# Neela08/cloud-security-pytorch-sagemaker-distributed-workshop

Hardware: AMD Instinct MI355X
Metric: images/sec (whole node) ResNet-50 DDP (higher is better)
Workload: dtype bf16; 1 GPU; model=resnet50, global_batch=256, per_gpu_batch=256, image_size=224, parallelism=dp1, optimizer=SGD(momentum=0.9, wd=1e-4), fp32 master weights, bf16 compute, backend=none, launcher=none, device=cuda, comm_forced_at_world1=False, buckets=5, grad_comm=fp32, wgrad_stream=True, hip_graph=False, gpu_max_hw_queues=8

## Files before the change

### csrc/kernels/norm_act.hip

```cpp
#include "common.h"
#include <mutex>
#include <algorithm>
#include <cstdlib>

namespace {

constexpr int NT = 256;
constexpr bool kBnxNt = false;

struct SlabGeom {
  int tpr;
  int rp;
  int cw;
};

__host__ __device__ inline SlabGeom slab_geom(int C) {
  SlabGeom g;
  g.tpr = C / 8 < NT ? C / 8 : NT;
  g.rp = NT / g.tpr;
  g.cw = g.tpr * 8;
  return g;
}

__device__ __forceinline__ void block_reduce_store(float* s0, float* s1, float* part, int C, int cbase,
                                                   const SlabGeom& g) {
  __shared__ float red[2][NT * 8];
  const int tid = threadIdx.x;
  const int c8 = tid % g.tpr, r0 = tid / g.tpr;
#pragma unroll
  for (int j = 0; j < 8; ++j) {
    red[0][r0 * g.cw + c8 * 8 + j] = s0[j];
// ... 735 lines not shown
    *(float4*)&b[0] = *(const float4*)(shift + cc); *(float4*)&b[4] = *(const float4*)(shift + cc + 4);
#pragma unroll
    for (int j = 0; j < 8; ++j) { best[j] = -INFINITY; bi[j] = 0; }
#pragma unroll
    for (int tp = 0; tp < 9; ++tp) {
      if (!ok[tp]) continue;
      float f[8];
      unpack8(v[tp], f);
#pragma unroll
      for (int j = 0; j < 8; ++j) {
        const float val = bf2f(f2bf(fmaxf(f[j] * a[j] + b[j], 0.f)));
        if (val > best[j]) { best[j] = val; bi[j] = tp; }
      }
    }
    const size_t o = (size_t)t * 8;
    *(uint4*)(y + o) = pack8(best);
    uint2 packed;
    packed.x = bi[0] | (bi[1] << 8) | (bi[2] << 16) | (bi[3] << 24);
    packed.y = bi[4] | (bi[5] << 8) | (bi[6] << 16) | (bi[7] << 24);
    *(uint2*)(idx + o) = packed;
  }
}

__device__ __forceinline__ uint32_t tap_of(const uint2& ii, int j) {
  return ((j < 4 ? ii.x : ii.y) >> (8 * (j & 3))) & 0xffu;
}

__device__ __forceinline__ void bnpool3_quad(const bf16_t* __restrict__ dy, const uint8_t* __restrict__ idx,
                                             const bf16_t* __restrict__ c, const float* a, const float* b, int n,
                                             int p, int q, int cc, int H, int W, int C, int P, int Q, float dz[4][8],
                                             float cv[4][8], bool valid[4]) {
  const bool pn = p + 1 < P, qn = q + 1 < Q;
  const size_t o00 = (((size_t)n * P + p) * Q + q) * C + cc;
  const size_t o01 = qn ? o00 + C : o00, o10 = pn ? o00 + (size_t)Q * C : o00;
  const size_t o11 = (pn && qn) ? o00 + (size_t)Q * C + C : o00;
  const uint4 g00 = epi_ld16<kBnxNt>(dy + o00), g01 = epi_ld16<kBnxNt>(dy + o01);
  const uint4 g10 = epi_ld16<kBnxNt>(dy + o10), g11 = epi_ld16<kBnxNt>(dy + o11);
  const uint2 i00 = *(const uint2*)(idx + o00), i01 = *(const uint2*)(idx + o01);
  const uint2 i10 = *(const uint2*)(idx + o10), i11 = *(const uint2*)(idx + o11);
  const int h0 = 2 * p, w0 = 2 * q;
  uint4 xv[4];
#pragma unroll
  for (int i = 0; i < 4; ++i) {
    const int h = h0 + (i >> 1), w = w0 + (i & 1);
    valid[i] = h < H && w < W;
    xv[i] = epi_ld16<kBnxNt>(c + (((size_t)n * H + (valid[i] ? h : h0)) * W + (valid[i] ? w : w0)) * C + cc);
  }
  float f00[8], f01[8], f10[8], f11[8];
  unpack8(g00, f00); unpack8(g01, f01); unpack8(g10, f10); unpack8(g11, f11);
#pragma unroll
  for (int i = 0; i < 4; ++i) unpack8(xv[i], cv[i]);
#pragma unroll
  for (int j = 0; j < 8; ++j) {
    const uint32_t t00 = tap_of(i00, j), t01 = qn ? tap_of(i01, j) : 0xffu;
    const uint32_t t10 = pn ? tap_of(i10, j) : 0xffu, t11 = (pn && qn) ? tap_of(i11, j) : 0xffu;
    float acc[4];
    acc[0] = t00 == 4u ? f00[j] : 0.f;
    acc[1] = (t00 == 5u ? f00[j] : 0.f) + (t01 == 3u ? f01[j] : 0.f);
    acc[2] = (t00 == 7u ? f00[j] : 0.f) + (t10 == 1u ? f10[j] : 0.f);
    acc[3] = (t00 == 8u ? f00[j] : 0.f) + (t01 == 6u ? f01[j] : 0.f) + (t10 == 2u ? f10[j] : 0.f) +
             (t11 == 0u ? f11[j] : 0.f);
#pragma unroll
    for (int i = 0; i < 4; ++i) dz[i][j] = bf2f(f2bf(cv[i][j] * a[j] + b[j])) > 0.f ? acc[i] : 0.f;
  }
}

__global__ __launch_bounds__(NT) void bnpool3_bwd_stats_kernel(const bf16_t* __restrict__ dy,
                                                               const uint8_t* __restrict__ idx,
                                                               const bf16_t* __restrict__ c,
                                                               const float* __restrict__ scale,
                                                               const float* __restrict__ shift,
                                                               const float* __restrict__ mean,
                                                               float* __restrict__ part, int Nb, int H, int W, int C,
                                                               int P, int Q, int rows_per_block) {
  const SlabGeom g = slab_geom(C);
  const int tid = threadIdx.x;
  const int c8 = tid % g.tpr, r0 = tid / g.tpr;
  const int cbase = blockIdx.y * g.cw;
  const int cc = cbase + c8 * 8;
  const int M = Nb * P * Q;
  const int rb = blockIdx.x * rows_per_block, re = min(M, rb + rows_per_block);
  float a[8], b[8], mu[8];
#pragma unroll
  for (int j = 0; j < 8; ++j) { a[j] = scale[cc + j]; b[j] = shift[cc + j]; mu[j] = mean[cc + j]; }
  float sd[8] = {0}, sq[8] = {0};
  for (int r = rb + r0; r < re; r += g.rp) {
    const int q = r % Q, np = r / Q;
    const int p = np % P, n = np / P;
    float dz[4][8], cv[4][8];
    bool valid[4];
    bnpool3_quad(dy, idx, c, a, b, n, p, q, cc, H, W, C, P, Q, dz, cv, valid);
#pragma unroll
    for (int i = 0; i < 4; ++i) {
      if (!valid[i]) continue;
#pragma unroll
      for (int j = 0; j < 8; ++j) { sd[j] += dz[i][j]; sq[j] += dz[i][j] * (cv[i][j] - mu[j]); }
    }
  }
  block_reduce_store(sd, sq, part, C, cbase, g);
}

__global__ __launch_bounds__(NT) void bnpool3_bwd_apply_kernel(const bf16_t* __restrict__ dy,
                                                               const uint8_t* __restrict__ idx,
                                                               const bf16_t* __restrict__ c,
                                                               const float* __restrict__ scale,
                                                               const float* __restrict__ shift,
                                                               const float* __restrict__ coef,
                                                               bf16_t* __restrict__ dc, int H, int W, int C, int P,
                                                               int Q, int total) {
  const int C8 = C / 8;
  for (int t = blockIdx.x * NT + threadIdx.x; t < total; t += gridDim.x * NT) {
    const int c8 = t % C8;
    const int pix = t / C8;
    const int q = pix % Q, np = pix / Q;
    const int p = np % P, n = np / P;
    const int cc = c8 * 8;
    float a[8], b[8], k0[8], k1[8], k2[8];
    *(float4*)&a[0] = *(const float4*)(scale + cc); *(float4*)&a[4] = *(const float4*)(scale + cc + 4);
    *(float4*)&b[0] = *(const float4*)(shift + cc); *(float4*)&b[4] = *(const float4*)(shift + cc + 4);
    *(float4*)&k0[0] = *(const float4*)(coef + cc); *(float4*)&k0[4] = *(const float4*)(coef + cc + 4);
    *(float4*)&k1[0] = *(const float4*)(coef + C + cc); *(float4*)&k1[4] = *(const float4*)(coef + C + cc + 4);
    *(float4*)&k2[0] = *(const float4*)(coef + 2 * C + cc); *(float4*)&k2[4] = *(const float4*)(coef + 2 * C + cc + 4);
    float dz[4][8], cv[4][8];
    bool valid[4];
    bnpool3_quad(dy, idx, c, a, b, n, p, q, cc, H, W, C, P, Q, dz, cv, valid);
#pragma unroll
    for (int i = 0; i < 4; ++i) {
      if (!valid[i]) continue;
      float o[8];
#pragma unroll
      for (int j = 0; j < 8; ++j) o[j] = k0[j] * dz[i][j] + k1[j] * cv[i][j] + k2[j];
      *(uint4*)(dc + (((size_t)n * H + 2 * p + (i >> 1)) * W + 2 * q + (i & 1)) * C + cc) = pack8(o);
    }
  }
}

inline int ew_grid_cap() {
  static int cap = -1;
  if (cap < 0) {
    const char* e = std::getenv("MI355X_DP_EW_GRID_CAP");
    cap = (e && std::atoi(e) > 0) ? std::atoi(e) : kEwGridCap;
  }
  return cap;
}

inline int ew_grid(int64_t nvec) {
  int64_t g = (nvec + NT * EW_U - 1) / (NT * EW_U);
  const int cap = ew_grid_cap();
  return (int)(g < cap ? g : cap);
}

inline bool ew_fixc(int grid, int C) { return ((int64_t)grid * NT * 8) % C == 0; }

template <bool RES_BN>
inline void launch_bn_apply(const void* x, const void* res, void* y, const float* scale, const float* shift,
// ... 437 lines not shown

MI_API int mi_bnpool_fwd(const void* c, const float* scale, const float* shift, void* y, void* idx, int Nb, int H,
                         int W, int C, int P, int Q, int k, int s, int pad, hipStream_t st) {
  if (C % 8 || k * k > 255) return (int)hipErrorInvalidValue;
  const int64_t total = (int64_t)Nb * P * Q * (C / 8);
  const int64_t g = std::min<int64_t>((total + NT - 1) / NT, 16384);
  if (k == 3 && s == 2 && pad == 1 && total < INT32_MAX && (int64_t)Nb * H * W * C < INT32_MAX * 8ll) {
    hipLaunchKernelGGL(bnpool3_fwd_kernel, dim3((int)g), dim3(NT), 0, st, (const bf16_t*)c, scale, shift,
                       (bf16_t*)y, (uint8_t*)idx, H, W, C, P, Q, (int)total);
    return (int)hipGetLastError();
  }
  hipLaunchKernelGGL(bnpool_fwd_kernel, dim3((int)g), dim3(NT), 0, st, (const bf16_t*)c, scale, shift, (bf16_t*)y,
                     (uint8_t*)idx, Nb, H, W, C, P, Q, k, s, pad);
  return (int)hipGetLastError();
}

MI_API int mi_bnpool_bwd(const void* dy, const void* idx, const void* c, void* dc, int Nb, int H, int W, int C, int P,
                         int Q, int k, int s, int pad, const float* scale, const float* shift, const float* gamma,
                         const float* save_mean, const float* save_invstd, float* dgamma, float* dbeta, float* coef,
                         float* part, hipStream_t st) {
  if (C % 8 || k * k > 255) return (int)hipErrorInvalidValue;
  const int M = Nb * H * W;
  const bool k3 = k == 3 && s == 2 && pad == 1 && (int64_t)M * C < INT32_MAX;
  int nblk, rpb; dim3 grid;
  bnpool_launch_dims(k3 ? Nb * P * Q : M, C, nblk, rpb, grid);
  if (k3)
    hipLaunchKernelGGL(bnpool3_bwd_stats_kernel, grid, dim3(NT), 0, st, (const bf16_t*)dy, (const uint8_t*)idx,
                       (const bf16_t*)c, scale, shift, save_mean, part, Nb, H, W, C, P, Q, rpb);
  else
    hipLaunchKernelGGL(bnpool_bwd_stats_kernel, grid, dim3(NT), 0, st, (const bf16_t*)dy, (const uint8_t*)idx,
                       (const bf16_t*)c, scale, shift, save_mean, part, Nb, H, W, C, P, Q, k, s, pad, rpb);
  slab_finalize<true>(part, nblk, fin_bwd_args(M, C, gamma, save_mean, save_invstd, dgamma, dbeta, coef), st);
  if (k3) {
    const int total3 = Nb * P * Q * (C / 8);
    hipLaunchKernelGGL(bnpool3_bwd_apply_kernel, dim3(std::min(cdiv(total3, NT), 16384)), dim3(NT), 0, st,
                       (const bf16_t*)dy, (const uint8_t*)idx, (const bf16_t*)c, scale, shift, coef, (bf16_t*)dc, H,
                       W, C, P, Q, total3);
    return (int)hipGetLastError();
  }
  const int64_t total = (int64_t)M * (C / 8);
  const int64_t g = std::min<int64_t>((total + NT - 1) / NT, 16384);
  hipLaunchKernelGGL(bnpool_bwd_apply_kernel, dim3((int)g), dim3(NT), 0, st, (const bf16_t*)dy, (const uint8_t*)idx,
                     (const bf16_t*)c, scale, shift, coef, (bf16_t*)dc, Nb, H, W, C, P, Q, k, s, pad);
  return (int)hipGetLastError();
}
```

### csrc/kernels/stem_conv.hip

```cpp
#include "common.h"
#include <algorithm>
#include <cstdlib>

extern "C" float* mi_partials_workspace(size_t floats, hipStream_t st);

namespace {

constexpr int SR = 7, SS = 7, SSTR = 2;
constexpr int NTAP = SR * SS;
constexpr int KSTEPS = (NTAP + 3) / 4;
constexpr int KOUT = 64;
constexpr int ROWPX = 256;
constexpr int PAIR_ROWS = SSTR + SR;
constexpr int NEW_ROWS = 2 * SSTR;
constexpr int NRING = PAIR_ROWS + NEW_ROWS;
constexpr int MAX_BLOCKS = 256;
constexpr int STEM_T = 512;

struct StemArgs {
  const bf16_t* x;
  const bf16_t* w;
  bf16_t* y;
  float* stats;
  int Nb, H, W, P, Q, pad;
// ... 152 lines not shown
  }
  __syncthreads();
  if (tid < 2 * KOUT) {
    const int which = tid / KOUT, n = tid - which * KOUT;
    float t = 0.f;
#pragma unroll
    for (int w8 = 0; w8 < 8; ++w8) t += sred[(w8 * 2 + which) * KOUT + n];
    a.stats[((size_t)blockIdx.x * 2 + which) * KOUT + n] = t;
  }
}

constexpr int NUT = (NTAP + 1) / 2;
constexpr int DYPX = 128;
constexpr int STEM_WELEMS = KOUT * NTAP * 8;

struct StemWArgs {
  const bf16_t* x;
  const bf16_t* dy;
  float* dw;
  float* ws;
  int Nb, H, W, P, Q, pad;
  int pairs_per_img, total_pairs, pairs_per_block;
  int x_bytes, dy_bytes;
};

__device__ __forceinline__ int dy_swz(int px) { return (((px >> 1) & 1) << 1) | (((px >> 3) & 1) << 2); }

__global__ __launch_bounds__(STEM_T, 1) void stem_wgrad_kernel(StemWArgs a) {
  extern __shared__ __attribute__((aligned(16))) uint4 sm[];
  uint4* ring = sm;
  uint4* dys = sm + NRING * ROWPX;

  const int tid = threadIdx.x, lane = tid & 63, wid = tid >> 6;
  const int g = lane >> 4, li = lane & 15, q4 = li >> 2, p4 = li & 3;
  const int g0 = blockIdx.x * a.pairs_per_block;
  const int g1 = min(a.total_pairs, g0 + a.pairs_per_block);
  const int HC = (a.Q - 1) * SSTR + SS;

  const __amdgpu_buffer_rsrc_t rsx = __builtin_amdgcn_make_buffer_rsrc((void*)a.x, (short)0, a.x_bytes, 0x00020000);
  const __amdgpu_buffer_rsrc_t rsd = __builtin_amdgcn_make_buffer_rsrc((void*)a.dy, (short)0, a.dy_bytes, 0x00020000);
  constexpr uint32_t OOB = 0xFFFFFFF0u;

  auto load_rows = [&](int img, int ih0, int nrows) {
    for (int c = wid; c < nrows * 4; c += 8) {
      const int k = c >> 2, part = c & 3;
      const int ih = ih0 + k;
      const int pos = part * 64 + lane;
      const int px = pos < ROWPX / 2 ? 2 * pos : 2 * (pos - ROWPX / 2) + 1;
      const int iw = px - a.pad;
      const bool ok = px < HC && (unsigned)ih < (unsigned)a.H && (unsigned)iw < (unsigned)a.W;
      const uint32_t vo = ok ? (uint32_t)((((img * a.H + ih) * a.W + iw) * 8) * 2) : OOB;
      const int slot = (ih + a.pad) % NRING;
      __builtin_amdgcn_raw_ptr_buffer_load_lds(rsx, LDS_PTR(void, &ring[slot * ROWPX + part * 64]), 16, vo, 0, 0, 0);
    }
  };
  auto load_dy = [&](int img, int jp, int buf) {
    for (int c = wid; c < 2 * DYPX / 8; c += 8) {
      const int h = c / (DYPX / 8), px = (c % (DYPX / 8)) * 8 + (lane >> 3);
      const int p = 2 * jp + h;
      const int lc = (lane & 7) ^ dy_swz(px);
      const bool ok = px < a.Q && p < a.P;
      const uint32_t vo = ok ? (uint32_t)((((img * a.P + p) * a.Q + px) * KOUT + lc * 8) * 2) : OOB;
      __builtin_amdgcn_raw_ptr_buffer_load_lds(rsd, LDS_PTR(void, &dys[((buf * 2 + h) * DYPX + (c % (DYPX / 8)) * 8) * 8]),
                                               16, vo, 0, 0, 0);
    }
  };

  f32x4 acc[4][4];
#pragma unroll
  for (int m = 0; m < 4; ++m)
#pragma unroll
    for (int v = 0; v < 4; ++v) acc[m][v] = f32x4{0.f, 0.f, 0.f, 0.f};
  const int nv = wid + 24 < NUT ? 4 : 3;

  if (g0 < g1) {
    const int img = g0 / a.pairs_per_img, j = g0 - img * a.pairs_per_img;
    load_rows(img, 2 * SSTR * j - a.pad, PAIR_ROWS);
    load_dy(img, j, 0);
  }
  int buf = 0;
  const uint2* ring2 = (const uint2*)ring;
  const uint2* dys2 = (const uint2*)dys;
  for (int gp = g0; gp < g1; ++gp) {
    const int img = gp / a.pairs_per_img, jp = gp - img * a.pairs_per_img;
    asm volatile("s_waitcnt vmcnt(0)" ::: "memory");
    __syncthreads();
    const bool next_same = gp + 1 < g1 && (gp + 1) / a.pairs_per_img == img;
    if (next_same) {
      load_rows(img, 2 * SSTR * jp - a.pad + PAIR_ROWS, NEW_ROWS);
      load_dy(img, jp + 1, buf ^ 1);
    }
#pragma unroll
    for (int h = 0; h < 2; ++h) {
      const int p = 2 * jp + h;
      if (p >= a.P) continue;
      const int rbase = (SSTR * p) % NRING;
      for (int c = 0; c < DYPX / 32; ++c) {
        if (32 * c >= a.Q) break;
        const int px1 = 32 * c + 8 * g + q4, px2 = px1 + 4;
        bf16x8 af[4], bfr[4];
#pragma unroll
        for (int m = 0; m < 4; ++m) {
          const int lc = 2 * m + (p4 >> 1);
          const uint2* r1 = dys2 + ((buf * 2 + h) * DYPX + px1) * 16 + 2 * (lc ^ dy_swz(px1)) + (p4 & 1);
          const uint2* r2 = dys2 + ((buf * 2 + h) * DYPX + px2) * 16 + 2 * (lc ^ dy_swz(px2)) + (p4 & 1);
          short4v lo = __builtin_amdgcn_ds_read_tr16_b64_v4i16(LDS_PTR(short4v, r1));
          short4v hi = __builtin_amdgcn_ds_read_tr16_b64_v4i16(LDS_PTR(short4v, r2));
          short v8 __attribute__((ext_vector_type(8))) = {lo[0], lo[1], lo[2], lo[3], hi[0], hi[1], hi[2], hi[3]};
          af[m] = __builtin_bit_cast(bf16x8, v8);
        }
        const int qa = min(px1, a.Q - 1), qb = min(px2, a.Q - 1);
#pragma unroll
        for (int v = 0; v < 4; ++v) {
          if (v >= nv) break;
          const int u = wid + 8 * v;
          const int t = min(2 * u + (p4 >> 1), NTAP - 1);
          const int r = t / SS, sx = t - (t / SS) * SS;
          int slot = rbase + r;
          slot = slot >= NRING ? slot - NRING : slot;
          const int cb = slot * ROWPX + (sx & 1) * (ROWPX / 2) + (sx >> 1);
          short4v lo = __builtin_amdgcn_ds_read_tr16_b64_v4i16(LDS_PTR(short4v, ring2 + (cb + qa) * 2 + (p4 & 1)));
          short4v hi = __builtin_amdgcn_ds_read_tr16_b64_v4i16(LDS_PTR(short4v, ring2 + (cb + qb) * 2 + (p4 & 1)));
          short v8 __attribute__((ext_vector_type(8))) = {lo[0], lo[1], lo[2], lo[3], hi[0], hi[1], hi[2], hi[3]};
          bfr[v] = __builtin_bit_cast(bf16x8, v8);
        }
#pragma unroll
        for (int v = 0; v < 4; ++v) {
          if (v >= nv) break;
#pragma unroll
          for (int m = 0; m < 4; ++m)
            acc[m][v] = __builtin_amdgcn_mfma_f32_16x16x32_bf16(af[m], bfr[v], acc[m][v], 0, 0, 0);
        }
      }
    }
    buf ^= 1;
    if (gp + 1 < g1 && !next_same) {
      asm volatile("s_waitcnt vmcnt(0)" ::: "memory");
      __syncthreads();
      const int img2 = (gp + 1) / a.pairs_per_img, j2 = (gp + 1) - img2 * a.pairs_per_img;
      load_rows(img2, 2 * SSTR * j2 - a.pad, PAIR_ROWS);
      load_dy(img2, j2, buf);
    }
  }
  float* prow = a.ws ? a.ws + (size_t)blockIdx.x * STEM_WELEMS : nullptr;
#pragma unroll
  for (int v = 0; v < 4; ++v) {
    if (v >= nv) break;
    const int tap = 2 * (wid + 8 * v) + (li >> 3);
    if (tap >= NTAP) continue;
#pragma unroll
    for (int m = 0; m < 4; ++m)
#pragma unroll
      for (int r = 0; r < 4; ++r) {
        const int k = 16 * m + 4 * g + r;
        const size_t o = ((size_t)k * NTAP + tap) * 8 + (li & 7);
        if (prow) prow[o] = acc[m][v][r];
        else atomicAdd(a.dw + o, acc[m][v][r]);
      }
  }
}

constexpr int SWR_POS = 32, SWR_G = 8;
__global__ __launch_bounds__(256) void stem_wgrad_reduce_kernel(const float4* __restrict__ ws, float4* __restrict__ dw,
                                                                int rows) {
// ... 38 lines not shown
      float v[8];
#pragma unroll
      for (int u = 0; u < 8; ++u) v[u] = b + u * SWR_G < rows ? ws[(size_t)(b + u * SWR_G) * STEM_WELEMS + o] : 0.f;
#pragma unroll
      for (int u = 0; u < 8; ++u) s += v[u];
    }
  red[grp][pl] = s;
  __syncthreads();
  if (grp != 0 || pos >= ne) return;
  for (int gg = 1; gg < SWR_G; ++gg) s += red[gg][pl];
  float* d = g + k * sK + c * sC + (tap / SS) * sR + (tap % SS) * sS;
  *d += s;
}

__global__ __launch_bounds__(256) void stem_wpack_kernel(const bf16_t* __restrict__ src, bf16_t* __restrict__ dst,
                                                         int total, int Cw, int R, int S, int64_t sK, int64_t sC,
                                                         int64_t sR, int64_t sS) {
  const int e = blockIdx.x * 256 + threadIdx.x;
  if (e >= total) return;
  const int c = e & 7, t = e >> 3, tap = t % (R * S), k = t / (R * S);
  dst[e] = c < Cw ? src[k * sK + c * sC + (tap / S) * sR + (tap % S) * sS] : (bf16_t)0;
}

constexpr size_t stem_wgrad_lds_bytes() { return (size_t)(NRING * ROWPX + 2 * 2 * DYPX * 8) * 16; }

constexpr size_t stem_lds_bytes() {
  return (size_t)(NRING * ROWPX) * 16 + 8 * 2 * KOUT * 4;
}

static int g_stem_blocks = -1;
inline int stem_blocks(int total_pairs) {
  if (g_stem_blocks < 0) {
    const char* e = std::getenv("MI355X_DP_STEM_BLOCKS");
    g_stem_blocks = e ? std::max(1, std::atoi(e)) : MAX_BLOCKS;
  }
  return std::max(1, std::min(total_pairs, g_stem_blocks));
}

}

MI_API int mi_stem_conv_ok(int C, int K, int R, int S, int stride, int pad, int Q) {
  return C == 8 && K == KOUT && R == SR && S == SS && stride == SSTR && pad >= 0 && pad < SR &&
         (Q - 1) * SSTR + SS <= ROWPX && Q <= 128;
}

MI_API int mi_stem_conv_stat_rows(int Nb, int P) { return stem_blocks(Nb * ((P + 1) / 2)); }

// ... 6 lines not shown
  a.x = (const bf16_t*)x; a.w = (const bf16_t*)w; a.y = (bf16_t*)y; a.stats = stats;
  a.Nb = Nb; a.H = H; a.W = W; a.P = P; a.Q = Q; a.pad = pad;
  a.pairs_per_img = (P + 1) / 2;
  a.total_pairs = Nb * a.pairs_per_img;
  const int blocks = stem_blocks(a.total_pairs);
  a.pairs_per_block = cdiv(a.total_pairs, blocks);
  a.x_bytes = (int)xb;
  static bool attr = false;
  if (!attr) {
    hipFuncSetAttribute((const void*)stem_conv_kernel, hipFuncAttributeMaxDynamicSharedMemorySize,
                        (int)stem_lds_bytes());
    attr = true;
  }
  hipLaunchKernelGGL(stem_conv_kernel, dim3(blocks), dim3(STEM_T), stem_lds_bytes(), st, a);
  return (int)hipGetLastError();
}

struct StemWTo {
  float* g;
  int Cw;
  int64_t sK, sC, sR, sS;
};

static int stem_wgrad_impl(const void* x, const void* dy, float* dw, const StemWTo* to, int Nb, int H, int W, int P,
                           int Q, int pad, hipStream_t st) {
  if (!mi_stem_conv_ok(8, KOUT, SR, SS, SSTR, pad, Q) || Q > DYPX) return (int)hipErrorInvalidValue;
  const int64_t xb = (int64_t)Nb * H * W * 8 * 2, db = (int64_t)Nb * P * Q * KOUT * 2;
  if (xb > 0x7FFFFFF0LL || db > 0x7FFFFFF0LL) return (int)hipErrorInvalidValue;
  StemWArgs a{};
  a.x = (const bf16_t*)x; a.dy = (const bf16_t*)dy; a.dw = dw;
  a.Nb = Nb; a.H = H; a.W = W; a.P = P; a.Q = Q; a.pad = pad;
  a.pairs_per_img = (P + 1) / 2;
  a.total_pairs = Nb * a.pairs_per_img;
  const int blocks = stem_blocks(a.total_pairs);
  a.pairs_per_block = cdiv(a.total_pairs, blocks);
  a.x_bytes = (int)xb;
  a.dy_bytes = (int)db;
  static int atomic_mode = -1;
  if (atomic_mode < 0) {
    const char* e = std::getenv("MI355X_DP_STEM_ATOMIC");
    atomic_mode = (e && e[0] == '1') ? 1 : 0;
  }
  a.ws = (!atomic_mode && ((uintptr_t)dw & 15) == 0) ? mi_partials_workspace((size_t)blocks * STEM_WELEMS, st)
                                                     : nullptr;
  static bool attr = false;
  if (!attr) {
    hipFuncSetAttribute((const void*)stem_wgrad_kernel, hipFuncAttributeMaxDynamicSharedMemorySize,
                        (int)stem_wgrad_lds_bytes());
    attr = true;
  }
  if (to && !a.ws) return (int)hipErrorNotSupported;
  hipLaunchKernelGGL(stem_wgrad_kernel, dim3(blocks), dim3(STEM_T), stem_wgrad_lds_bytes(), st, a);
  if (to)
    hipLaunchKernelGGL(stem_wgrad_reduce_to_kernel, dim3(cdiv(KOUT * NTAP * to->Cw, SWR_POS)), dim3(256), 0, st,
                       (const float*)a.ws, to->g, blocks, to->Cw, to->sK, to->sC, to->sR, to->sS);
  else if (a.ws)
    hipLaunchKernelGGL(stem_wgrad_reduce_kernel, dim3(cdiv(STEM_WELEMS / 4, SWR_POS)), dim3(256), 0, st,
                       (const float4*)a.ws, (float4*)dw, blocks);
  return (int)hipGetLastError();
}

MI_API int mi_stem_wgrad(const void* x, const void* dy, float* dw, int Nb, int H, int W, int P, int Q, int pad,
                         hipStream_t st) {
  return stem_wgrad_impl(x, dy, dw, nullptr, Nb, H, W, P, Q, pad, st);
}

MI_API int mi_stem_wgrad_to(const void* x, const void* dy, float* g, int Cw, int64_t sK, int64_t sC, int64_t sR,
                            int64_t sS, int Nb, int H, int W, int K, int R, int S, int stride, int P, int Q, int pad,
                            hipStream_t st) {
  if (Cw < 1 || Cw > 8) return (int)hipErrorInvalidValue;
  const char* e = std::getenv("MI355X_DP_STEM_KERNEL");
  if ((e && e[0] == '0') || !mi_stem_conv_ok(8, K, R, S, stride, pad, Q)) return (int)hipErrorNotSupported;
  if (P != (H + 2 * pad - R) / stride + 1 || Q != (W + 2 * pad - S) / stride + 1) return (int)hipErrorInvalidValue;
  const StemWTo to{g, Cw, sK, sC, sR, sS};
  return stem_wgrad_impl(x, dy, nullptr, &to, Nb, H, W, P, Q, pad, st);
}

MI_API int mi_stem_wpack(const void* src, void* dst, int K, int Cw, int R, int S, int64_t sK, int64_t sC, int64_t sR,
                         int64_t sS, hipStream_t st) {
  if (K < 1 || R < 1 || S < 1 || Cw < 1 || Cw > 8 || (int64_t)K * R * S * 8 > 0x7FFFFFFF)
    return (int)hipErrorInvalidValue;
  const int total = K * R * S * 8;
  hipLaunchKernelGGL(stem_wpack_kernel, dim3(cdiv(total, 256)), dim3(256), 0, st, (const bf16_t*)src, (bf16_t*)dst,
                     total, Cw, R, S, sK, sC, sR, sS);
  return (int)hipGetLastError();
}
```

### mi355x_dp/ops/kernels.py

```python
from ._lib import signature, c_void_p as P, c_int as I, c_int64 as L, c_float as F
import ctypes

U32 = ctypes.c_uint32

signature("mi_conv2d_fwd", P, P, P, P, P, I, I, I, I, I, I, I, I, I, I, I, I, P)
signature("mi_set_glds", I)
signature("mi_set_nt_stages", I)
signature("mi_set_nt_split_blocks", I)
signature("mi_set_nt_split_fused", I)
signature("mi_set_tn_split_fused", I)
signature("mi_set_tn_stages", I)
signature("mi_conv2d_dgrad", P, P, P, I, I, I, I, I, I, I, I, I, I, I, P)
signature("mi_conv2d_wgrad", P, P, P, I, I, I, I, I, I, I, I, I, I, I, P)
signature("mi_conv_nol_ok", I, I, I, I, I, I, I, I, I, I, I)
signature("mi_conv2d_fwd_nol", P, P, P, P, P, P, I, I, I, I, I, I, I, I, I, I, I, P)
signature("mi_conv2d_wgrad_nol", P, P, P, P, P, I, I, I, I, I, I, I, I, I, I, I, P)
signature("mi_conv2d_dgrad_ex3", P, P, P, I, I, I, I, I, I, I, I, I, I, I, I, P, P, P, I, P, I, P, P, P)
signature("mi_conv2d_dgrad_ex4", P, P, P, I, I, I, I, I, I, I, I, I, I, I, I, P, P, P, I, P, I, P, P, P, P)
signature("mi_set_gemm256", I)
signature("mi_set_conv256_min_tiles", I)
signature("mi_set_conv256_min_k", I)
signature("mi_set_panel_first", I)
signature("mi_set_wgrad256", I)
signature("mi_set_ds256", I)
signature("mi_conv_stat_rows_g", I, I, I, I, I, I, I, I, I, I, I)
signature("mi_conv_stat_rows", I, I, I, I)
signature("mi_dgrad_stat_rows_g", I, I, I, I, I, I, I, I, I, I, I)
signature("mi_dgrad_stat_rows", I, I, I, I, I, I, I, I, I)
signature("mi_conv_fbb_route", I, I, I)
signature("mi_conv_fbb_rows", I, I, I)
signature("mi_conv2d_dgrad_ex", P, P, P, I, I, I, I, I, I, I, I, I, I, I, I, P, P, P, I, P, P)
signature("mi_conv2d_dgrad_ex2", P, P, P, I, I, I, I, I, I, I, I, I, I, I, I, P, P, P, I, P, I, P)
signature("mi_conv_wtrans", P, P, I, I, I, P)
signature("mi_stem_wpack", P, P, I, I, I, I, L, L, L, L, P)
signature("mi_stem_wgrad_to", P, P, P, I, L, L, L, L, I, I, I, I, I, I, I, I, I, I, P)
signature("mi_conv_wtrans_multi", P, P, P, I, I, P)
signature("mi_gemm_nt", P, P, P, P, P, I, I, I, I, I, I, I, I, P)
signature("mi_gemm_tn", P, P, P, I, I, I, I, I, I, P)
signature("mi_gemm_tn_bias", P, P, P, P, I, I, I, I, I, I, P)
signature("mi_register_wgrad_stream", P)
signature("mi_register_aux_stream", P)
signature("mi_create_cu_masked_stream", I, I, P)
signature("mi_splitk_ws_reserve", ctypes.c_size_t, P)

signature("mi_bn_partial_rows", I, I)
signature("mi_bn_slab_extra_rows")
signature("mi_bn_set_small_elems", L)
signature("mi_bn_init_counters")
signature("mi_bn_fwd_train", P, P, P, I, I, F, F, P, P, P, P, P, P, P, P, P, P, I, I, P)
signature("mi_bn_apply_dual", P, P, P, I, I, P, P, P, P, I, P)
signature("mi_bn_apply_bits", P, P, P, P, I, I, P, P, P, P, P)
signature("mi_bn_fwd_eval", P, P, P, I, I, F, P, P, P, P, P, P, I, P)
signature("mi_bn_bwd_train", P, P, P, P, P, I, I, P, P, P, P, P, P, P, I, P)
signature("mi_bn_bwd_eval", P, P, P, P, P, I, I, I, P)
signature("mi_bnpool_partial_rows", I, I)
signature("mi_bnpool_fwd", P, P, P, P, P, I, I, I, I, I, I, I, I, I, P)
signature("mi_bnpool_bwd", P, P, P, P, I, I, I, I, I, I, I, I, I, P, P, P, P, P, P, P, P, P, P)

# ... 121 lines not shown
```

### mi355x_dp/ops/stem.py

```python
from __future__ import annotations

import torch

from . import _lib
from . import kernels as _k
from ._lib import ptr, stream_of
from .functional import BF16, CL, _finish_grad, _grad_buffer, _nhwc, pad_channels8, weight_bf16

F32 = torch.float32


def _out(h, r, s, p):
    return (h + 2 * p - r) // s + 1


class _Stem(torch.autograd.Function):
    @staticmethod
    def forward(ctx, x, geom, wconv, gamma, beta, rmean, rvar, nbt, momentum, eps):
        stride, pad, pk, ps, pp = geom
        N, C, H, W = x.shape
        K, Cw, R, S = wconv.shape
        P, Q = _out(H, R, stride, pad), _out(W, S, stride, pad)
        P2, Q2 = _out(P, pk, ps, pp), _out(Q, pk, ps, pp)
        dev = x.device
# ... 16 lines not shown
        y = torch.empty((N, K, P2, Q2), dtype=BF16, device=dev, memory_format=CL)
        idx = torch.empty((N, P2, Q2, K), dtype=torch.uint8, device=dev)
        _lib.call("mi_bnpool_fwd", ptr(c), ptr(scale), ptr(shift), ptr(y), ptr(idx), N, P, Q, K, P2, Q2, pk, ps, pp,
                  st)
        ctx.save_for_backward(x, c, idx, mean, invstd, scale, shift)
        ctx.params = (wconv, gamma, beta)
        ctx.geom = (N, H, W, K, Cw, R, S, stride, pad, P, Q, P2, Q2, pk, ps, pp)
        return y

    @staticmethod
    def backward(ctx, dy):
        x, c, idx, mean, invstd, scale, shift = ctx.saved_tensors
        wconv, gamma, beta = ctx.params
        N, H, W, K, Cw, R, S, stride, pad, P, Q, P2, Q2, pk, ps, pp = ctx.geom
        dy = _nhwc(dy)
        dev = dy.device
        st = stream_of(dy)
        lib = _lib.load()
        gw, gb = _grad_buffer(gamma), _grad_buffer(beta)
        M = N * P * Q
        rows = max(lib.mi_bnpool_partial_rows(M, K), lib.mi_bnpool_partial_rows(N * P2 * Q2, K))
        part = torch.empty((rows + lib.mi_bn_slab_extra_rows(), 2, K), dtype=F32, device=dev)
        coef = torch.empty((3, K), dtype=F32, device=dev)
        dc = torch.empty_like(c, memory_format=CL)
        _lib.call("mi_bnpool_bwd", ptr(dy), ptr(idx), ptr(c), ptr(dc), N, P, Q, K, P2, Q2, pk, ps, pp, ptr(scale),
                  ptr(shift), ptr(gamma), ptr(mean), ptr(invstd), ptr(gw), ptr(gb), ptr(coef), ptr(part), st)
        dgamma, dbeta = _finish_grad(gamma, gw), _finish_grad(beta, gb)
        g = _grad_buffer(wconv)
        rc = lib.mi_stem_wgrad_to(ptr(x), ptr(dc), ptr(g), Cw, *g.stride(), N, H, W, K, R, S, stride, P, Q, pad, st)
        if rc != 0:
            gp = torch.zeros((K, R, S, 8), dtype=F32, device=dev)
            _lib.call("mi_conv2d_wgrad", ptr(x), ptr(dc), ptr(gp), N, H, W, 8, K, R, S, stride, pad, P, Q, st)
            g.add_(gp[..., :Cw].permute(0, 3, 1, 2))
        dw = _finish_grad(wconv, g)
        return None, None, dw, dgamma, dbeta, None, None, None, None, None


def fusable(conv, bn, pool, x) -> bool:
    from mi355x_dp.models.layers import BatchNorm2d, Conv2d, MaxPool2d
    if not (x.is_cuda and x.dtype == BF16 and torch.is_grad_enabled() and bn.training and not x.requires_grad):
        return False
    if not (isinstance(conv, Conv2d) and isinstance(bn, BatchNorm2d) and isinstance(pool, MaxPool2d)):
        return False
    if conv.bias is not None or conv.groups != 1 or conv.in_channels > 8 or conv.out_channels % 8 != 0:
        return False
    if len(set(conv.stride)) != 1 or len(set(conv.padding)) != 1 or conv.dilation not in ((1, 1), 1):
        return False
    if not bn.track_running_stats or not bn.affine or bn.momentum is None:
        return False
    ks = pool.kernel_size if isinstance(pool.kernel_size, int) else pool.kernel_size[0]
    if pool.ceil_mode or pool.dilation not in (1, (1, 1)) or ks * ks > 255:
# ... 13 lines not shown
```

Before: 13980 images/s.

## Fuse stem BN/maxpool backward apply into stem wgrad kernel

The stem's BN+ReLU+maxpool backward apply step, which wrote a full-resolution dc tensor, is now computed inside the stem weight-gradient kernel. Each block derives the dc tile on the fly from dy, the pool indices and c, and stages it into LDS in place of loading a precomputed dc. This removes one kernel launch and a full write and read of the largest activation gradient. The stats kernel is also software-pipelined with double-buffered loads and scheduling barriers. The cost is more ALU and register pressure in the wgrad kernel and extra LDS for the per-channel coefficients.

```diff
diff --git a/csrc/kernels/bnpool3.h b/csrc/kernels/bnpool3.h
--- /dev/null
+++ b/csrc/kernels/bnpool3.h
@@ -0,0 +1,88 @@
+#pragma once
+#include "common.h"
+
+constexpr bool kBnxNt = false;
+
+__device__ __forceinline__ uint32_t tap_of(const uint2& ii, int j) {
+  return ((j < 4 ? ii.x : ii.y) >> (8 * (j & 3))) & 0xffu;
+}
+
+struct Bnpool3Raw {
+  uint4 g00, g01, g10, g11;
+  uint2 i00, i01, i10, i11;
+  uint4 xv[4];
+};
+
+__device__ __forceinline__ void bnpool3_load(const bf16_t* __restrict__ dy, const uint8_t* __restrict__ idx,
+                                             const bf16_t* __restrict__ c, int n, int p, int q, int cc, int H, int W,
+                                             int C, int P, int Q, Bnpool3Raw& r) {
+  const bool pn = p + 1 < P, qn = q + 1 < Q;
+  const size_t o00 = (((size_t)n * P + p) * Q + q) * C + cc;
+  const size_t o01 = qn ? o00 + C : o00, o10 = pn ? o00 + (size_t)Q * C : o00;
+  const size_t o11 = (pn && qn) ? o00 + (size_t)Q * C + C : o00;
+  r.g00 = epi_ld16<kBnxNt>(dy + o00); r.g01 = epi_ld16<kBnxNt>(dy + o01);
+  r.g10 = epi_ld16<kBnxNt>(dy + o10); r.g11 = epi_ld16<kBnxNt>(dy + o11);
+  r.i00 = *(const uint2*)(idx + o00); r.i01 = *(const uint2*)(idx + o01);
+  r.i10 = *(const uint2*)(idx + o10); r.i11 = *(const uint2*)(idx + o11);
+  const int h0 = 2 * p, w0 = 2 * q;
+#pragma unroll
+  for (int i = 0; i < 4; ++i) {
+    const int h = h0 + (i >> 1), w = w0 + (i & 1);
+    const bool in = h < H && w < W;
+    r.xv[i] = epi_ld16<kBnxNt>(c + (((size_t)n * H + (in ? h : h0)) * W + (in ? w : w0)) * C + cc);
+  }
+}
+
+__device__ __forceinline__ void bnpool3_dz1(float f00, float f01, float f10, float f11, uint32_t t00, uint32_t t01,
+                                            uint32_t t10, uint32_t t11, const float cv[4], float a, float b,
+                                            float dz[4]) {
+  float acc[4];
+  acc[0] = t00 == 4u ? f00 : 0.f;
+  acc[1] = (t00 == 5u ? f00 : 0.f) + (t01 == 3u ? f01 : 0.f);
+  acc[2] = (t00 == 7u ? f00 : 0.f) + (t10 == 1u ? f10 : 0.f);
+  acc[3] = (t00 == 8u ? f00 : 0.f) + (t01 == 6u ? f01 : 0.f) + (t10 == 2u ? f10 : 0.f) + (t11 == 0u ? f11 : 0.f);
+#pragma unroll
+  for (int i = 0; i < 4; ++i) dz[i] = bf2f(f2bf(__builtin_fmaf(cv[i], a, b))) > 0.f ? acc[i] : 0.f;
+}
+
+__device__ __forceinline__ float bnpool3_dc1(float k0, float k1, float k2, float dz, float cv) {
+  return __builtin_fmaf(k0, dz, k1 * cv) + k2;
+}
+
+__device__ __forceinline__ void bnpool3_dz(const Bnpool3Raw& r, const float* a, const float* b, int p, int q, int H,
+                                           int W, int P, int Q, float dz[4][8], float cv[4][8], bool valid[4]) {
+  const bool pn = p + 1 < P, qn = q + 1 < Q;
+#pragma unroll
+  for (int i = 0; i < 4; ++i) valid[i] = 2 * p + (i >> 1) < H && 2 * q + (i & 1) < W;
+  float f00[8], f01[8], f10[8], f11[8];
+  unpack8(r.g00, f00); unpack8(r.g01, f01); unpack8(r.g10, f10); unpack8(r.g11, f11);
+#pragma unroll
+  for (int i = 0; i < 4; ++i) unpack8(r.xv[i], cv[i]);
+#pragma unroll
+  for (int j = 0; j < 8; ++j) {
+    const uint32_t t00 = tap_of(r.i00, j), t01 = qn ? tap_of(r.i01, j) : 0xffu;
+    const uint32_t t10 = pn ? tap_of(r.i10, j) : 0xffu, t11 = (pn && qn) ? tap_of(r.i11, j) : 0xffu;
+    const float cj[4] = {cv[0][j], cv[1][j], cv[2][j], cv[3][j]};
+    float dj[4];
+    bnpool3_dz1(f00[j], f01[j], f10[j], f11[j], t00, t01, t10, t11, cj, a[j], b[j], dj);
+#pragma unroll
+    for (int i = 0; i < 4; ++i) dz[i][j] = dj[i];
+  }
+}
+
+__device__ __forceinline__ void bnpool3_quad(const bf16_t* __restrict__ dy, const uint8_t* __restrict__ idx,
+                                             const bf16_t* __restrict__ c, const float* a, const float* b, int n,
+                                             int p, int q, int cc, int H, int W, int C, int P, int Q, float dz[4][8],
+                                             float cv[4][8], bool valid[4]) {
+  Bnpool3Raw r;
+  bnpool3_load(dy, idx, c, n, p, q, cc, H, W, C, P, Q, r);
+  bnpool3_dz(r, a, b, p, q, H, W, P, Q, dz, cv, valid);
+}
+
+__device__ __forceinline__ uint4 bnpool3_dc(const float* k0, const float* k1, const float* k2, const float* dz,
+                                            const float* cv) {
+  float o[8];
+#pragma unroll
+  for (int j = 0; j < 8; ++j) o[j] = bnpool3_dc1(k0[j], k1[j], k2[j], dz[j], cv[j]);
+  return pack8(o);
+}
diff --git a/csrc/kernels/norm_act.hip b/csrc/kernels/norm_act.hip
--- a/csrc/kernels/norm_act.hip
+++ b/csrc/kernels/norm_act.hip
@@ -1,4 +1,5 @@
 #include "common.h"
+#include "bnpool3.h"
 #include <mutex>
 #include <algorithm>
 #include <cstdlib>
@@ -6,7 +7,6 @@
 namespace {
 
 constexpr int NT = 256;
-constexpr bool kBnxNt = false;
 
 struct SlabGeom {
   int tpr;
@@ -788,48 +788,6 @@
   }
 }
 
-__device__ __forceinline__ uint32_t tap_of(const uint2& ii, int j) {
-  return ((j < 4 ? ii.x : ii.y) >> (8 * (j & 3))) & 0xffu;
-}
-
-__device__ __forceinline__ void bnpool3_quad(const bf16_t* __restrict__ dy, const uint8_t* __restrict__ idx,
-                                             const bf16_t* __restrict__ c, const float* a, const float* b, int n,
-                                             int p, int q, int cc, int H, int W, int C, int P, int Q, float dz[4][8],
-                                             float cv[4][8], bool valid[4]) {
-  const bool pn = p + 1 < P, qn = q + 1 < Q;
-  const size_t o00 = (((size_t)n * P + p) * Q + q) * C + cc;
-  const size_t o01 = qn ? o00 + C : o00, o10 = pn ? o00 + (size_t)Q * C : o00;
-  const size_t o11 = (pn && qn) ? o00 + (size_t)Q * C + C : o00;
-  const uint4 g00 = epi_ld16<kBnxNt>(dy + o00), g01 = epi_ld16<kBnxNt>(dy + o01);
-  const uint4 g10 = epi_ld16<kBnxNt>(dy + o10), g11 = epi_ld16<kBnxNt>(dy + o11);
-  const uint2 i00 = *(const uint2*)(idx + o00), i01 = *(const uint2*)(idx + o01);
-  const uint2 i10 = *(const uint2*)(idx + o10), i11 = *(const uint2*)(idx + o11);
-  const int h0 = 2 * p, w0 = 2 * q;
-  uint4 xv[4];
-#pragma unroll
-  for (int i = 0; i < 4; ++i) {
-    const int h = h0 + (i >> 1), w = w0 + (i & 1);
-    valid[i] = h < H && w < W;
-    xv[i] = epi_ld16<kBnxNt>(c + (((size_t)n * H + (valid[i] ? h : h0)) * W + (valid[i] ? w : w0)) * C + cc);
-  }
-  float f00[8], f01[8], f10[8], f11[8];
-  unpack8(g00, f00); unpack8(g01, f01); unpack8(g10, f10); unpack8(g11, f11);
-#pragma unroll
-  for (int i = 0; i < 4; ++i) unpack8(xv[i], cv[i]);
-#pragma unroll
-  for (int j = 0; j < 8; ++j) {
-    const uint32_t t00 = tap_of(i00, j), t01 = qn ? tap_of(i01, j) : 0xffu;
-    const uint32_t t10 = pn ? tap_of(i10, j) : 0xffu, t11 = (pn && qn) ? tap_of(i11, j) : 0xffu;
-    float acc[4];
-    acc[0] = t00 == 4u ? f00[j] : 0.f;
-    acc[1] = (t00 == 5u ? f00[j] : 0.f) + (t01 == 3u ? f01[j] : 0.f);
-    acc[2] = (t00 == 7u ? f00[j] : 0.f) + (t10 == 1u ? f10[j] : 0.f);
-    acc[3] = (t00 == 8u ? f00[j] : 0.f) + (t01 == 6u ? f01[j] : 0.f) + (t10 == 2u ? f10[j] : 0.f) +
-             (t11 == 0u ? f11[j] : 0.f);
-#pragma unroll
-    for (int i = 0; i < 4; ++i) dz[i][j] = bf2f(f2bf(cv[i][j] * a[j] + b[j])) > 0.f ? acc[i] : 0.f;
-  }
-}
 
 __global__ __launch_bounds__(NT) void bnpool3_bwd_stats_kernel(const bf16_t* __restrict__ dy,
                                                                const uint8_t* __restrict__ idx,
@@ -850,17 +808,35 @@
 #pragma unroll
   for (int j = 0; j < 8; ++j) { a[j] = scale[cc + j]; b[j] = shift[cc + j]; mu[j] = mean[cc + j]; }
   float sd[8] = {0}, sq[8] = {0};
-  for (int r = rb + r0; r < re; r += g.rp) {
+  auto fetch = [&](int r, int fallback, Bnpool3Raw& raw) {
+    r = r < re ? r : fallback;
     const int q = r % Q, np = r / Q;
-    const int p = np % P, n = np / P;
+    bnpool3_load(dy, idx, c, np / P, np % P, q, cc, H, W, C, P, Q, raw);
+  };
+  auto consume = [&](const Bnpool3Raw& raw, int r, int fallback) {
+    const bool live = r < re;
+    r = live ? r : fallback;
+    const int q = r % Q, p = (r / Q) % P;
     float dz[4][8], cv[4][8];
     bool valid[4];
-    bnpool3_quad(dy, idx, c, a, b, n, p, q, cc, H, W, C, P, Q, dz, cv, valid);
+    bnpool3_dz(raw, a, b, p, q, H, W, P, Q, dz, cv, valid);
 #pragma unroll
     for (int i = 0; i < 4; ++i) {
-      if (!valid[i]) continue;
+      if (!valid[i] || !live) continue;
 #pragma unroll
       for (int j = 0; j < 8; ++j) { sd[j] += dz[i][j]; sq[j] += dz[i][j] * (cv[i][j] - mu[j]); }
+    }
+  };
+  if (rb + r0 < re) {
+    Bnpool3Raw A, B;
+    fetch(rb + r0, rb + r0, A);
+    for (int r = rb + r0; r < re; r += 2 * g.rp) {
+      fetch(r + g.rp, r, B);
+      __builtin_amdgcn_sched_barrier(0);
+      consume(A, r, r);
+      fetch(r + 2 * g.rp, r, A);
+      __builtin_amdgcn_sched_barrier(0);
+      consume(B, r + g.rp, r);
     }
   }
   block_reduce_store(sd, sq, part, C, cbase, g);
@@ -893,10 +869,8 @@
 #pragma unroll
     for (int i = 0; i < 4; ++i) {
       if (!valid[i]) continue;
-      float o[8];
-#pragma unroll
-      for (int j = 0; j < 8; ++j) o[j] = k0[j] * dz[i][j] + k1[j] * cv[i][j] + k2[j];
-      *(uint4*)(dc + (((size_t)n * H + 2 * p + (i >> 1)) * W + 2 * q + (i & 1)) * C + cc) = pack8(o);
+      *(uint4*)(dc + (((size_t)n * H + 2 * p + (i >> 1)) * W + 2 * q + (i & 1)) * C + cc) =
+          bnpool3_dc(k0, k1, k2, dz[i], cv[i]);
     }
   }
 }
@@ -1380,6 +1354,7 @@
   if (C % 8 || k * k > 255) return (int)hipErrorInvalidValue;
   const int M = Nb * H * W;
   const bool k3 = k == 3 && s == 2 && pad == 1 && (int64_t)M * C < INT32_MAX;
+  if (!dc && !k3) return (int)hipErrorInvalidValue;
   int nblk, rpb; dim3 grid;
   bnpool_launch_dims(k3 ? Nb * P * Q : M, C, nblk, rpb, grid);
   if (k3)
@@ -1390,6 +1365,7 @@
                        (const bf16_t*)c, scale, shift, save_mean, part, Nb, H, W, C, P, Q, k, s, pad, rpb);
   slab_finalize<true>(part, nblk, fin_bwd_args(M, C, gamma, save_mean, save_invstd, dgamma, dbeta, coef), st);
   if (k3) {
+    if (!dc) return (int)hipGetLastError();
     const int total3 = Nb * P * Q * (C / 8);
     hipLaunchKernelGGL(bnpool3_bwd_apply_kernel, dim3(std::min(cdiv(total3, NT), 16384)), dim3(NT), 0, st,
                        (const bf16_t*)dy, (const uint8_t*)idx, (const bf16_t*)c, scale, shift, coef, (bf16_t*)dc, H,
diff --git a/csrc/kernels/stem_conv.hip b/csrc/kernels/stem_conv.hip
--- a/csrc/kernels/stem_conv.hip
+++ b/csrc/kernels/stem_conv.hip
@@ -1,4 +1,5 @@
 #include "common.h"
+#include "bnpool3.h"
 #include <algorithm>
 #include <cstdlib>
 
@@ -198,14 +199,21 @@
   int Nb, H, W, P, Q, pad;
   int pairs_per_img, total_pairs, pairs_per_block;
   int x_bytes, dy_bytes;
+  const bf16_t* dyp;
+  const uint8_t* idx;
+  const bf16_t* c;
+  const float *scale, *shift, *coef;
+  int P2, Q2;
 };
 
 __device__ __forceinline__ int dy_swz(int px) { return (((px >> 1) & 1) << 1) | (((px >> 3) & 1) << 2); }
 
+template <bool FUSED>
 __global__ __launch_bounds__(STEM_T, 1) void stem_wgrad_kernel(StemWArgs a) {
   extern __shared__ __attribute__((aligned(16))) uint4 sm[];
   uint4* ring = sm;
   uint4* dys = sm + NRING * ROWPX;
+  float* cst = (float*)(dys + 2 * 2 * DYPX * 8);
 
   const int tid = threadIdx.x, lane = tid & 63, wid = tid >> 6;
   const int g = lane >> 4, li = lane & 15, q4 = li >> 2, p4 = li & 3;
@@ -242,6 +250,63 @@
     }
   };
 
+  const int fo = tid & 7, fq2 = tid >> 3;
+  const bool factive = FUSED && fq2 < a.Q2;
+  Bnpool3Raw raw = {};
+  auto fetch_quad = [&](int img, int jp) {
+    if (factive) bnpool3_load(a.dyp, a.idx, a.c, img, jp, fq2, fo * 8, a.P, a.Q, KOUT, a.P2, a.Q2, raw);
+  };
+  auto stage_quad = [&](int jp, int buf) {
+    const bool pn = jp + 1 < a.P2, qn = fq2 + 1 < a.Q2;
+    bool valid[4];
+#pragma unroll
+    for (int i = 0; i < 4; ++i) valid[i] = factive && 2 * jp + (i >> 1) < a.P && 2 * fq2 + (i & 1) < a.Q;
+    uint2* st[4];
+#pragma unroll
+    for (int i = 0; i < 4; ++i) {
+      const int px = 2 * fq2 + (i & 1);
+      st[i] = (uint2*)(dys + ((buf * 2 + (i >> 1)) * DYPX + px) * 8 + (fo ^ dy_swz(px)));
+    }
+#pragma unroll 1
+    for (int hh = 0; hh < 2; ++hh) {
+      const uint4 gs[4] = {raw.g00, raw.g01, raw.g10, raw.g11};
+      float f[4][4], cv[4][4];
+#pragma unroll
+      for (int k = 0; k < 4; ++k) {
+        const uint32_t g0w = hh ? gs[k].z : gs[k].x, g1w = hh ? gs[k].w : gs[k].y;
+        f[k][0] = __uint_as_float(g0w << 16); f[k][1] = __uint_as_float(g0w & 0xffff0000u);
+        f[k][2] = __uint_as_float(g1w << 16); f[k][3] = __uint_as_float(g1w & 0xffff0000u);
+        const uint32_t c0w = hh ? raw.xv[k].z : raw.xv[k].x, c1w = hh ? raw.xv[k].w : raw.xv[k].y;
+        cv[k][0] = __uint_as_float(c0w << 16); cv[k][1] = __uint_as_float(c0w & 0xffff0000u);
+        cv[k][2] = __uint_as_float(c1w << 16); cv[k][3] = __uint_as_float(c1w & 0xffff0000u);
+      }
+      const uint32_t w00 = hh ? raw.i00.y : raw.i00.x;
+      const uint32_t w01 = qn ? (hh ? raw.i01.y : raw.i01.x) : 0xffffffffu;
+      const uint32_t w10 = pn ? (hh ? raw.i10.y : raw.i10.x) : 0xffffffffu;
+      const uint32_t w11 = (pn && qn) ? (hh ? raw.i11.y : raw.i11.x) : 0xffffffffu;
+      const float* cs = cst + fo * 8 + 4 * hh;
+      const float4 sa = *(const float4*)(cs), sb = *(const float4*)(cs + KOUT);
+      const float4 k0 = *(const float4*)(cs + 2 * KOUT), k1 = *(const float4*)(cs + 3 * KOUT);
+      const float4 k2 = *(const float4*)(cs + 4 * KOUT);
+      const float sav[4] = {sa.x, sa.y, sa.z, sa.w}, sbv[4] = {sb.x, sb.y, sb.z, sb.w};
+      const float k0v[4] = {k0.x, k0.y, k0.z, k0.w}, k1v[4] = {k1.x, k1.y, k1.z, k1.w};
+      const float k2v[4] = {k2.x, k2.y, k2.z, k2.w};
+      float o[4][4];
+#pragma unroll
+      for (int j = 0; j < 4; ++j) {
+        const float cj[4] = {cv[0][j], cv[1][j], cv[2][j], cv[3][j]};
+        float dj[4];
+        bnpool3_dz1(f[0][j], f[1][j], f[2][j], f[3][j], (w00 >> (8 * j)) & 0xffu, (w01 >> (8 * j)) & 0xffu,
+                    (w10 >> (8 * j)) & 0xffu, (w11 >> (8 * j)) & 0xffu, cj, sav[j], sbv[j], dj);
+#pragma unroll
+        for (int i = 0; i < 4; ++i) o[i][j] = bnpool3_dc1(k0v[j], k1v[j], k2v[j], dj[i], cj[i]);
+      }
+#pragma unroll
+      for (int i = 0; i < 4; ++i)
+        st[i][hh] = valid[i] ? make_uint2(pack2bf(o[i][0], o[i][1]), pack2bf(o[i][2], o[i][3])) : make_uint2(0u, 0u);
+    }
+  };
+
   f32x4 acc[4][4];
 #pragma unroll
   for (int m = 0; m < 4; ++m)
@@ -249,22 +314,30 @@
     for (int v = 0; v < 4; ++v) acc[m][v] = f32x4{0.f, 0.f, 0.f, 0.f};
   const int nv = wid + 24 < NUT ? 4 : 3;
 
+  if (FUSED) {
+    for (int u = tid; u < 5 * KOUT; u += STEM_T)
+      cst[u] = u < KOUT ? a.scale[u] : u < 2 * KOUT ? a.shift[u - KOUT] : a.coef[u - 2 * KOUT];
+    __syncthreads();
+  }
   if (g0 < g1) {
     const int img = g0 / a.pairs_per_img, j = g0 - img * a.pairs_per_img;
     load_rows(img, 2 * SSTR * j - a.pad, PAIR_ROWS);
-    load_dy(img, j, 0);
+    if (FUSED) { fetch_quad(img, j); stage_quad(j, 0); }
+    else load_dy(img, j, 0);
   }
   int buf = 0;
   const uint2* ring2 = (const uint2*)ring;
   const uint2* dys2 = (const uint2*)dys;
   for (int gp = g0; gp < g1; ++gp) {
     const int img = gp / a.pairs_per_img, jp = gp - img * a.pairs_per_img;
-    asm volatile("s_waitcnt vmcnt(0)" ::: "memory");
+    if (FUSED) asm volatile("s_waitcnt vmcnt(0) lgkmcnt(0)" ::: "memory");
+    else asm volatile("s_waitcnt vmcnt(0)" ::: "memory");
     __syncthreads();
     const bool next_same = gp + 1 < g1 && (gp + 1) / a.pairs_per_img == img;
     if (next_same) {
       load_rows(img, 2 * SSTR * jp - a.pad + PAIR_ROWS, NEW_ROWS);
-      load_dy(img, jp + 1, buf ^ 1);
+      if (FUSED) fetch_quad(img, jp + 1);
+      else load_dy(img, jp + 1, buf ^ 1);
     }
 #pragma unroll
     for (int h = 0; h < 2; ++h) {
@@ -309,13 +382,16 @@
         }
       }
     }
+    if (FUSED && next_same) stage_quad(jp + 1, buf ^ 1);
     buf ^= 1;
     if (gp + 1 < g1 && !next_same) {
-      asm volatile("s_waitcnt vmcnt(0)" ::: "memory");
+      const int img2 = (gp + 1) / a.pairs_per_img, j2 = (gp + 1) - img2 * a.pairs_per_img;
+      if (FUSED) fetch_quad(img2, j2);
+      else asm volatile("s_waitcnt vmcnt(0)" ::: "memory");
       __syncthreads();
-      const int img2 = (gp + 1) / a.pairs_per_img, j2 = (gp + 1) - img2 * a.pairs_per_img;
       load_rows(img2, 2 * SSTR * j2 - a.pad, PAIR_ROWS);
-      load_dy(img2, j2, buf);
+      if (FUSED) stage_quad(j2, buf);
+      else load_dy(img2, j2, buf);
     }
   }
   float* prow = a.ws ? a.ws + (size_t)blockIdx.x * STEM_WELEMS : nullptr;
@@ -400,7 +476,9 @@
   dst[e] = c < Cw ? src[k * sK + c * sC + (tap / S) * sR + (tap % S) * sS] : (bf16_t)0;
 }
 
-constexpr size_t stem_wgrad_lds_bytes() { return (size_t)(NRING * ROWPX + 2 * 2 * DYPX * 8) * 16; }
+constexpr size_t stem_wgrad_lds_bytes(bool fused) {
+  return (size_t)(NRING * ROWPX + 2 * 2 * DYPX * 8) * 16 + (fused ? 5 * KOUT * 4 : 0);
+}
 
 constexpr size_t stem_lds_bytes() {
   return (size_t)(NRING * ROWPX) * 16 + 8 * 2 * KOUT * 4;
@@ -453,13 +531,34 @@
   int64_t sK, sC, sR, sS;
 };
 
+struct StemWPool {
+  const void *dyp, *idx, *c;
+  const float *scale, *shift, *coef;
+  int P2, Q2;
+};
+
+static bool stem_wgrad_atomic() {
+  static int atomic_mode = -1;
+  if (atomic_mode < 0) {
+    const char* e = std::getenv("MI355X_DP_STEM_ATOMIC");
+    atomic_mode = (e && e[0] == '1') ? 1 : 0;
+  }
+  return atomic_mode != 0;
+}
+
 static int stem_wgrad_impl(const void* x, const void* dy, float* dw, const StemWTo* to, int Nb, int H, int W, int P,
-                           int Q, int pad, hipStream_t st) {
+                           int Q, int pad, hipStream_t st, const StemWPool* fp = nullptr) {
   if (!mi_stem_conv_ok(8, KOUT, SR, SS, SSTR, pad, Q) || Q > DYPX) return (int)hipErrorInvalidValue;
   const int64_t xb = (int64_t)Nb * H * W * 8 * 2, db = (int64_t)Nb * P * Q * KOUT * 2;
   if (xb > 0x7FFFFFF0LL || db > 0x7FFFFFF0LL) return (int)hipErrorInvalidValue;
+  if (fp && (int64_t)Nb * fp->P2 * fp->Q2 * KOUT * 2 > 0x7FFFFFF0LL) return (int)hipErrorInvalidValue;
   StemWArgs a{};
   a.x = (const bf16_t*)x; a.dy = (const bf16_t*)dy; a.dw = dw;
+  if (fp) {
+    a.dyp = (const bf16_t*)fp->dyp; a.idx = (const uint8_t*)fp->idx; a.c = (const bf16_t*)fp->c;
+    a.scale = fp->scale; a.shift = fp->shift; a.coef = fp->coef;
+    a.P2 = fp->P2; a.Q2 = fp->Q2;
+  }
   a.Nb = Nb; a.H = H; a.W = W; a.P = P; a.Q = Q; a.pad = pad;
   a.pairs_per_img = (P + 1) / 2;
   a.total_pairs = Nb * a.pairs_per_img;
@@ -467,21 +566,21 @@
   a.pairs_per_block = cdiv(a.total_pairs, blocks);
   a.x_bytes = (int)xb;
   a.dy_bytes = (int)db;
-  static int atomic_mode = -1;
-  if (atomic_mode < 0) {
-    const char* e = std::getenv("MI355X_DP_STEM_ATOMIC");
-    atomic_mode = (e && e[0] == '1') ? 1 : 0;
-  }
-  a.ws = (!atomic_mode && ((uintptr_t)dw & 15) == 0) ? mi_partials_workspace((size_t)blocks * STEM_WELEMS, st)
-                                                     : nullptr;
+  a.ws = (!stem_wgrad_atomic() && ((uintptr_t)dw & 15) == 0) ? mi_partials_workspace((size_t)blocks * STEM_WELEMS, st)
+                                                             : nullptr;
   static bool attr = false;
   if (!attr) {
-    hipFuncSetAttribute((const void*)stem_wgrad_kernel, hipFuncAttributeMaxDynamicSharedMemorySize,
-                        (int)stem_wgrad_lds_bytes());
+    hipFuncSetAttribute((const void*)stem_wgrad_kernel<false>, hipFuncAttributeMaxDynamicSharedMemorySize,
+                        (int)stem_wgrad_lds_bytes(false));
+    hipFuncSetAttribute((const void*)stem_wgrad_kernel<true>, hipFuncAttributeMaxDynamicSharedMemorySize,
+                        (int)stem_wgrad_lds_bytes(true));
     attr = true;
   }
   if (to && !a.ws) return (int)hipErrorNotSupported;
-  hipLaunchKernelGGL(stem_wgrad_kernel, dim3(blocks), dim3(STEM_T), stem_wgrad_lds_bytes(), st, a);
+  if (fp)
+    hipLaunchKernelGGL(stem_wgrad_kernel<true>, dim3(blocks), dim3(STEM_T), stem_wgrad_lds_bytes(true), st, a);
+  else
+    hipLaunchKernelGGL(stem_wgrad_kernel<false>, dim3(blocks), dim3(STEM_T), stem_wgrad_lds_bytes(false), st, a);
   if (to)
     hipLaunchKernelGGL(stem_wgrad_reduce_to_kernel, dim3(cdiv(KOUT * NTAP * to->Cw, SWR_POS)), dim3(256), 0, st,
                        (const float*)a.ws, to->g, blocks, to->Cw, to->sK, to->sC, to->sR, to->sS);
@@ -507,6 +606,46 @@
   return stem_wgrad_impl(x, dy, nullptr, &to, Nb, H, W, P, Q, pad, st);
 }
 
+static int g_stem_fused_bwd = -1;
+static bool stem_fused_bwd() {
+  if (g_stem_fused_bwd < 0) {
+    const char* e = std::getenv("MI355X_DP_STEM_FUSED_BWD");
+    g_stem_fused_bwd = (e && e[0] == '0') ? 0 : 1;
+  }
+  return g_stem_fused_bwd != 0;
+}
+
+MI_API int mi_set_stem_fused_bwd(int on) {
+  g_stem_fused_bwd = on < 0 ? -1 : on ? 1 : 0;
+  return 0;
+}
+
+MI_API int mi_stem_wgrad_lds_bytes(int fused) { return (int)stem_wgrad_lds_bytes(fused != 0); }
+
+MI_API int mi_stem_wgrad_bnpool_ok(int Nb, int H, int W, int K, int R, int S, int stride, int P, int Q, int pad,
+                                   int pk, int ps, int pp, int P2, int Q2, hipStream_t st) {
+  const char* e = std::getenv("MI355X_DP_STEM_KERNEL");
+  if (!stem_fused_bwd() || (e && e[0] == '0') || stem_wgrad_atomic()) return 0;
+  if (Nb < 1 || !mi_stem_conv_ok(8, K, R, S, stride, pad, Q) || Q > DYPX) return 0;
+  if (P != (H + 2 * pad - R) / stride + 1 || Q != (W + 2 * pad - S) / stride + 1) return 0;
+  if (pk != 3 || ps != 2 || pp != 1 || P2 != (P + 1) / 2 || Q2 != (Q + 1) / 2) return 0;
+  const int64_t xb = (int64_t)Nb * H * W * 8 * 2, cb = (int64_t)Nb * P * Q * KOUT * 2;
+  if (xb > 0x7FFFFFF0LL || cb > 0x7FFFFFF0LL) return 0;
+  return mi_partials_workspace((size_t)stem_blocks(Nb * ((P + 1) / 2)) * STEM_WELEMS, st) != nullptr;
+}
+
+MI_API int mi_stem_wgrad_bnpool_to(const void* x, const void* dyp, const void* idx, const void* c, const float* scale,
+                                   const float* shift, const float* coef, float* g, int Cw, int64_t sK, int64_t sC,
+                                   int64_t sR, int64_t sS, int Nb, int H, int W, int K, int R, int S, int stride,
+                                   int P, int Q, int pad, int pk, int ps, int pp, int P2, int Q2, hipStream_t st) {
+  if (Cw < 1 || Cw > 8) return (int)hipErrorInvalidValue;
+  if (!mi_stem_wgrad_bnpool_ok(Nb, H, W, K, R, S, stride, P, Q, pad, pk, ps, pp, P2, Q2, st))
+    return (int)hipErrorNotSupported;
+  const StemWTo to{g, Cw, sK, sC, sR, sS};
+  const StemWPool fp{dyp, idx, c, scale, shift, coef, P2, Q2};
+  return stem_wgrad_impl(x, nullptr, nullptr, &to, Nb, H, W, P, Q, pad, st, &fp);
+}
+
 MI_API int mi_stem_wpack(const void* src, void* dst, int K, int Cw, int R, int S, int64_t sK, int64_t sC, int64_t sR,
                          int64_t sS, hipStream_t st) {
   if (K < 1 || R < 1 || S < 1 || Cw < 1 || Cw > 8 || (int64_t)K * R * S * 8 > 0x7FFFFFFF)
diff --git a/mi355x_dp/ops/kernels.py b/mi355x_dp/ops/kernels.py
--- a/mi355x_dp/ops/kernels.py
+++ b/mi355x_dp/ops/kernels.py
@@ -34,6 +34,11 @@
 signature("mi_conv_wtrans", P, P, I, I, I, P)
 signature("mi_stem_wpack", P, P, I, I, I, I, L, L, L, L, P)
 signature("mi_stem_wgrad_to", P, P, P, I, L, L, L, L, I, I, I, I, I, I, I, I, I, I, P)
+signature("mi_stem_wgrad_bnpool_ok", I, I, I, I, I, I, I, I, I, I, I, I, I, I, I, P)
+signature("mi_stem_wgrad_bnpool_to", P, P, P, P, P, P, P, P, I, L, L, L, L, I, I, I, I, I, I, I, I, I, I, I, I, I, I,
+          I, P)
+signature("mi_set_stem_fused_bwd", I)
+signature("mi_stem_wgrad_lds_bytes", I)
 signature("mi_conv_wtrans_multi", P, P, P, I, I, P)
 signature("mi_gemm_nt", P, P, P, P, P, I, I, I, I, I, I, I, I, P)
 signature("mi_gemm_tn", P, P, P, I, I, I, I, I, I, P)
diff --git a/mi355x_dp/ops/stem.py b/mi355x_dp/ops/stem.py
--- a/mi355x_dp/ops/stem.py
+++ b/mi355x_dp/ops/stem.py
@@ -62,11 +62,16 @@
         rows = max(lib.mi_bnpool_partial_rows(M, K), lib.mi_bnpool_partial_rows(N * P2 * Q2, K))
         part = torch.empty((rows + lib.mi_bn_slab_extra_rows(), 2, K), dtype=F32, device=dev)
         coef = torch.empty((3, K), dtype=F32, device=dev)
-        dc = torch.empty_like(c, memory_format=CL)
+        fused = lib.mi_stem_wgrad_bnpool_ok(N, H, W, K, R, S, stride, P, Q, pad, pk, ps, pp, P2, Q2, st) == 1
+        dc = None if fused else torch.empty_like(c, memory_format=CL)
         _lib.call("mi_bnpool_bwd", ptr(dy), ptr(idx), ptr(c), ptr(dc), N, P, Q, K, P2, Q2, pk, ps, pp, ptr(scale),
                   ptr(shift), ptr(gamma), ptr(mean), ptr(invstd), ptr(gw), ptr(gb), ptr(coef), ptr(part), st)
         dgamma, dbeta = _finish_grad(gamma, gw), _finish_grad(beta, gb)
         g = _grad_buffer(wconv)
+        if fused:
+            _lib.call("mi_stem_wgrad_bnpool_to", ptr(x), ptr(dy), ptr(idx), ptr(c), ptr(scale), ptr(shift),
+                      ptr(coef), ptr(g), Cw, *g.stride(), N, H, W, K, R, S, stride, P, Q, pad, pk, ps, pp, P2, Q2, st)
+            return None, None, _finish_grad(wconv, g), dgamma, dbeta, None, None, None, None, None
         rc = lib.mi_stem_wgrad_to(ptr(x), ptr(dc), ptr(g), Cw, *g.stride(), N, H, W, K, R, S, stride, P, Q, pad, st)
         if rc != 0:
             gp = torch.zeros((K, R, S, 8), dtype=F32, device=dev)
```

After: 14020 images/s (median of 6 runs). Within noise of the previous version (+0.3%).
